# lazear/sage

Measured on NVIDIA H100. Metric: spectra/sec, higher is better.
Workload: dtype f32

## Files before the change

### sage_b200/csrc/device_common.cuh

```cuda
#pragma once
#include <cuda_runtime.h>
#include <stdint.h>

namespace sb {

constexpr int K_MAX = 128;
constexpr uint32_t NARROW_CAP = 8192;
constexpr int PRELIM_THREADS = 256;
constexpr int SCORE_THREADS = 128;
#ifndef SAGE_B200_SCORE_MIN_CTAS
#define SAGE_B200_SCORE_MIN_CTAS 10
#endif
constexpr int SCORE_MIN_CTAS = SAGE_B200_SCORE_MIN_CTAS;
#ifndef SAGE_B200_SCORE_TILE
#define SAGE_B200_SCORE_TILE 1024
#endif
#ifndef SAGE_B200_SCORE_UNROLL
#define SAGE_B200_SCORE_UNROLL 1
#endif
#ifndef SAGE_B200_SCORE_MIN_CTAS_SPLIT
#define SAGE_B200_SCORE_MIN_CTAS_SPLIT 11
#endif
constexpr int SCORE_MIN_CTAS_SPLIT = SAGE_B200_SCORE_MIN_CTAS_SPLIT;
constexpr uint32_t SCORE_UNROLL = SAGE_B200_SCORE_UNROLL;
constexpr uint32_t SCORE_TILE = SAGE_B200_SCORE_TILE;
constexpr int MAX_KINDS = 6;
constexpr uint32_t WARPQ_CAP = 1024;
constexpr int WARPQ_WARPS = 2;
constexpr int WARPQ_MIN_CTAS = 24;
constexpr uint32_t PEP_LUT_CELLS = 65536;
constexpr uint32_t BUCKET_LUT_CELLS = 32768;

constexpr float PROTON = 1.0072764f;
constexpr float NEUTRON = 1.00335f;

struct Tol { int kind; float lo, hi; };

__device__ __forceinline__ int f32_key(float x) {
// ... 209 lines not shown
```

### sage_b200/csrc/kernels.cuh

```cuda
#pragma once
#include <type_traits>

#include "device_common.cuh"
#include "glibc_log.cuh"

#ifndef SAGE_B200_RARE_NOINLINE
#define SAGE_B200_RARE_NOINLINE 0
#endif
#if SAGE_B200_RARE_NOINLINE
#define SB_RARE __noinline__
#else
#define SB_RARE __forceinline__
#endif

namespace sb {

__device__ __forceinline__ uint32_t pep_partition(const DbView& db, float x, bool le) {
    uint32_t lo = 0, hi = db.n_pep;
    if (db.pep_lut != nullptr) {
        const float t = (x - db.plut_base) * db.plut_inv_w;
        if (t == t) {
            const int c = (int)fminf(fmaxf(floorf(t), -2.0f), (float)PEP_LUT_CELLS + 2.0f);
            lo = __ldg(db.pep_lut + min(max(c - 1, 0), (int)PEP_LUT_CELLS));
            hi = __ldg(db.pep_lut + min(max(c + 2, 0), (int)PEP_LUT_CELLS));
// ... 1294 lines not shown
    const int klo = f32_key(lo), khi = f32_key(hi);
    uint32_t i, j;
    binary_search_slice(n, [&](uint32_t k) { return f32_key(masses[k]) < klo; }, [&](uint32_t k) { return f32_key(masses[k]) <= khi; }, i, j);
    int best = -1;
    float max_int = 0.0f;
    for (uint32_t idx = i; idx < j; idx++) {
        const float m = masses[idx];
        if (m >= lo && m <= hi) {
            const float it = intens[idx];
            if (it >= max_int) { max_int = it; best = (int)idx; }
        }
    }
    return best;
}
__device__ __forceinline__ int select_most_intense_peak_lut(const float* masses, const float* intens, uint32_t n, float center, const Tol& tol,
                                                            const LutParams& LP, const uint16_t* lut) {
    float lo, hi;
    tol_bounds(tol, center, lo, hi);
    lo = __fadd_rn(lo, 0.0f);
    hi = __fadd_rn(hi, 0.0f);
    uint32_t idx = lut_start(LP, lut, lo, SPEC_LUT_CELLS);
    while (idx < n && masses[idx] < lo) idx++;
    int best = -1;
    float max_int = 0.0f;
    while (idx < n) {
        const float m = masses[idx];
        if (!(m <= hi)) break;
        const float it = intens[idx];
        if (it >= max_int) { max_int = it; best = (int)idx; }
        idx++;
    }
    return best;
}

__device__ __forceinline__ double ref_ln(const ScorerView& sc, double x) { return glog::glibc_log_v(x, (int)sc.log_variant); }
__device__ __forceinline__ double lnfact(const ScorerView& sc, uint32_t n) {
// ... 150 lines not shown

__device__ __forceinline__ unsigned long long f64_sort_key(double d) {
    const unsigned long long u = (unsigned long long)__double_as_longlong(d + 0.0);
    return (u >> 63) ? ~u : (u | 0x8000000000000000ull);
}
__device__ __forceinline__ double f64_from_sort_key(unsigned long long k) {
    const unsigned long long u = (k >> 63) ? (k & 0x7FFFFFFFFFFFFFFFull) : ~k;
    return __longlong_as_double((long long)u);
}

#if SAGE_B200_PHASE_CLOCKS
__device__ unsigned long long g_phase[16];
__shared__ long long s_ph_prev;
#define PH_START() do { if (threadIdx.x == 0) s_ph_prev = clock64(); } while (0)
#define PH(i) do { if (threadIdx.x == 0) { const long long n_ = clock64(); atomicAdd(&g_phase[i], (unsigned long long)(n_ - s_ph_prev)); s_ph_prev = n_; } } while (0)
#else
#define PH_START() do {} while (0)
#define PH(i) do {} while (0)
#endif

struct ScoreTile {
    CandHdr hdr[K_MAX + 1];
    double hkey[K_MAX];
    float term[SCORE_TILE];
    float inten[SCORE_TILE];
    uint32_t mask[SCORE_TILE / 32];
    uint16_t hits[SCORE_TILE];
    uint16_t lut[SPEC_LUT_CELLS];
    uint32_t scan[SCORE_THREADS / 32];
    unsigned long long hit_base;
    uint32_t hit_room;
};

__device__ __forceinline__ uint32_t kind_index(uint32_t ki, uint32_t nions) {
    uint32_t kind = ki >= nions;
    uint32_t idx = ki - (kind ? nions : 0);
    while (idx >= nions) { idx -= nions; kind++; }
    return kind << 13 | idx;
}

__device__ __forceinline__ bool fast_task(float ion, uint32_t fc, float tlo, float thi, const SpecView& sp, const uint16_t* lut, const float* pm, float& mz,
                                          uint32_t& idx) {
    const float q3 = __fmul_rn(ion, 1.0f / 3.0f);
    const float third = __fmaf_rn(__fmaf_rn(-q3, 3.0f, ion), 1.0f / 3.0f, q3);
    mz = fc == 1 ? ion : (fc == 2 ? __fmul_rn(ion, 0.5f) : third);
    const float pl = __fmul_rn(mz, tlo), ph = __fmul_rn(mz, thi);
    const float ql = __fmul_rn(pl, 1.0f / 1000000.0f), qh = __fmul_rn(ph, 1.0f / 1000000.0f);
    const float lo = __fadd_rn(mz, __fmaf_rn(__fmaf_rn(-ql, 1000000.0f, pl), 1.0f / 1000000.0f, ql));
    const float hi = __fadd_rn(mz, __fmaf_rn(__fmaf_rn(-qh, 1000000.0f, ph), 1.0f / 1000000.0f, qh));
    const float tt = __fmul_rn(__fsub_rn(lo, sp.lp.base), sp.lp.inv_w);
    const int cc = tt > 1.0f ? (int)fminf(tt, (float)(SPEC_LUT_CELLS - 1)) - 1 : 0;
    idx = lut[cc];
    while (pm[idx] < lo) idx++;
    return pm[idx] <= hi;
}

template <bool FAST, bool SPLIT>
__device__ __forceinline__ void score_candidates_flat(const DbView& db, const ScorerView& sc, const uint64_t* cur, uint32_t ncand, const SpecView& sp,
                                                      ScoreTile& S, ScoreRec* recs, const SplitOut& so, uint32_t spec) {
    const uint32_t tid = threadIdx.x, lane = tid & 31, warp = tid >> 5, nwarps = SCORE_THREADS / 32;
    constexpr uint32_t tile = SCORE_TILE;
    uint64_t key = 0;
    uint32_t L = 0, nions = 0, nfc = 1, total = 0, ion_off = 0;
    if (tid < ncand) {
        key = cur[tid];
        const uint32_t pep = key_peptide(key);
        L = __ldg(db.pep_len + pep);
        nions = L - 1;
        nfc = max_fragment_charge(sc.max_fragment_charge_opt, key_charge(key)) - 1;
        total = nions * nfc * db.n_kinds;
        ion_off = __ldg(db.ion_off + pep);
    }
    uint32_t incl = total;
#pragma unroll
    for (int o = 1; o < 32; o <<= 1) {
        const uint32_t v = __shfl_up_sync(0xffffffffu, incl, o);
        if (lane >= (uint32_t)o) incl += v;
    }
    if (lane == 31) S.scan[warp] = incl;
    __syncthreads();
    uint32_t base = incl - total, T = 0;
#pragma unroll
    for (uint32_t w = 0; w < nwarps; w++) {
        const uint32_t x = S.scan[w];
        if (w < warp) base += x;
        T += x;
    }
    if (tid < ncand) { CandHdr h; h.ion_off = ion_off; h.base = base; h.next = base + total; h.nions = (uint16_t)nions; h.nfc = (uint8_t)nfc; h.pad = 0; S.hdr[tid] = h; }
    if (tid == 0) { CandHdr h; h.ion_off = 0; h.base = T; h.next = 0xFFFFFFFFu; h.nions = 0; h.nfc = 1; h.pad = 0; S.hdr[ncand] = h; }
    uint32_t hcnt = 0, hits_before = 0;
    if (SPLIT && tid == 0) {
        const unsigned long long hb = atomicAdd(so.counters + C_HITS, (unsigned long long)T);
        const bool room = hb + T <= so.hit_cap;
        S.hit_base = hb;
        S.hit_room = room ? 1u : 0u;
        so.meta[spec].hit_base = hb;
        if (!room) so.meta[spec].ncand = 0;
    }
    uint32_t mb = 0, my = 0;
    float sb = 0.f, sy = 0.f, ppm = 0.f;
    Run brun = {0, 0, 0, 0}, yrun = {0, 0, 0, 0};
    const float tlo = sc.fragment_tol.lo, thi = sc.fragment_tol.hi;
    const float* const pm = sp.masses;
    const float* const pi = sp.intens;
    auto generic_task = [&](const CandHdr& h, uint32_t f, uint32_t slot) -> bool {
        uint32_t ki, fc;
        switch (h.nfc) {
            case 1: ki = f; fc = 1; break;
            case 2: ki = f >> 1; fc = (f & 1) + 1; break;
            case 3: ki = f / 3; fc = f - ki * 3 + 1; break;
            default: ki = f / h.nfc; fc = f - ki * h.nfc + 1; break;
        }
        const float ion = __ldg(db.ions + h.ion_off + ki);
        const float mz = fc == 1 ? ion : (fc == 2 && fabsf(ion) >= 1e-30f) ? __fmul_rn(ion, 0.5f) : __fdiv_rn(ion, (float)fc);
        const int pk = sp.use_lut ? select_most_intense_peak_lut(pm, pi, sp.np, mz, sc.fragment_tol, sp.lp, S.lut)
                                  : select_most_intense_peak(pm, pi, sp.np, mz, sc.fragment_tol);
        if (pk < 0) return false;
        const float peak_mass = pm[pk], inten = pi[pk];
        S.term[slot] = __fdiv_rn(__fmul_rn(__fmul_rn(inten, fabsf(__fsub_rn(mz, peak_mass))), 2E6f), __fadd_rn(mz, peak_mass));
        S.inten[slot] = inten;
        return true;
    };
    for (uint32_t t0 = 0; t0 < T; t0 += tile) {
        const uint32_t tn = min(tile, T - t0);
        __syncthreads();
        PH(t0 == 0 ? 3 : 5);
        constexpr uint32_t STEP = 32 * SCORE_UNROLL;
        const uint32_t chunk = (((tn + nwarps - 1) / nwarps) + STEP - 1) & ~(STEP - 1);
        const uint32_t w_lo = min(tn, warp * chunk), w_hi = min(tn, w_lo + chunk);
        uint32_t c = 0, wcount = 0;
        CandHdr h = S.hdr[0];
        if (w_lo < w_hi) {
            const uint32_t t_first = t0 + min(w_lo + lane, w_hi - 1);
            uint32_t lo = 0, hi = ncand;
            while (hi - lo > 1) { const uint32_t mid = (lo + hi) >> 1; if (S.hdr[mid].base <= t_first) lo = mid; else hi = mid; }
            c = lo;
            h = S.hdr[c];
// ... 15 lines not shown
                hB = h; fB = t - h.base;
            }
            if (FAST) {
                const bool okA = inA && hA.nfc <= 3, okB = inB && hB.nfc <= 3;
                const uint32_t kiA = hA.nfc == 1 ? fA : (hA.nfc == 2 ? fA >> 1 : __umulhi(fA, 0xAAAAAAABu) >> 1);
                const uint32_t kiB = hB.nfc == 1 ? fB : (hB.nfc == 2 ? fB >> 1 : __umulhi(fB, 0xAAAAAAABu) >> 1);
                const float ionA = okA ? __ldg(db.ions + hA.ion_off + kiA) : 0.0f;
                const float ionB = okB ? __ldg(db.ions + hB.ion_off + kiB) : 0.0f;
                const bool fastA = okA && ionA >= 1.0f && ionA <= 1e20f, fastB = okB && ionB >= 1.0f && ionB <= 1e20f;
                float mzA = 0.f, mzB = 0.f;
                uint32_t idxA = 0, idxB = 0;
                if (fastA) hitA = fast_task(ionA, fA - kiA * hA.nfc + 1, tlo, thi, sp, S.lut, pm, mzA, idxA);
                if (fastB) hitB = fast_task(ionB, fB - kiB * hB.nfc + 1, tlo, thi, sp, S.lut, pm, mzB, idxB);
                if (hitA) { S.term[slotA] = mzA; S.inten[slotA] = __uint_as_float(idxA); }
                if (hitB) { S.term[slotB] = mzB; S.inten[slotB] = __uint_as_float(idxB); }
                if (inA && !fastA) hitA = finalA = generic_task(hA, fA, slotA);
                if (inB && !fastB) hitB = finalB = generic_task(hB, fB, slotB);
            } else {
                if (inA) hitA = generic_task(hA, fA, slotA);
                if (inB) hitB = generic_task(hB, fB, slotB);
            }
            const uint32_t ballA = __ballot_sync(0xffffffffu, hitA), ballB = __ballot_sync(0xffffffffu, hitB);
            if (lane == 0) { S.mask[s0 >> 5] = ballA; if (SCORE_UNROLL == 2) S.mask[(s0 >> 5) + 1] = ballB; }
            if (FAST) {
                const uint32_t lt = (1u << lane) - 1;
                if (hitA) S.hits[w_lo + wcount + __popc(ballA & lt)] = (uint16_t)(slotA | (finalA ? 0x8000u : 0u));
                wcount += __popc(ballA);
                if (SCORE_UNROLL == 2) {
                    if (hitB) S.hits[w_lo + wcount + __popc(ballB & lt)] = (uint16_t)(slotB | (finalB ? 0x8000u : 0u));
                    wcount += __popc(ballB);
                }
            }
        }
        if (FAST) {
            __syncwarp();
// ... 12 lines not shown
                    const float it = pi[idx];
                    if (it >= max_int) { max_int = it; best = (int)idx; }
                    m = pm[++idx];
                } while (m <= hi);
                if (best >= 0) {
                    const float peak_mass = pm[best];
                    S.term[slot] = __fdiv_rn(__fmul_rn(__fmul_rn(max_int, fabsf(__fsub_rn(mz, peak_mass))), 2E6f), __fadd_rn(mz, peak_mass));
                    S.inten[slot] = max_int;
                } else {
                    atomicAnd(&S.mask[slot >> 5], ~(1u << (slot & 31)));
                }
            }
        }
        __syncthreads();
        PH(4);
        if (SPLIT) {
            const uint32_t nwords = (tn + 31) >> 5;
            const uint32_t mw = lane < nwords ? S.mask[lane] : 0u;
            uint32_t incl = (uint32_t)__popc(mw);
#pragma unroll
            for (int o = 1; o < 32; o <<= 1) {
                const uint32_t v = __shfl_up_sync(0xffffffffu, incl, o);
                if (lane >= (uint32_t)o) incl += v;
            }
            const uint32_t pre = incl - (uint32_t)__popc(mw), tile_total = __shfl_sync(0xffffffffu, incl, 31);
            const uint32_t word = tid >> 2, q8 = (tid & 3) * 8;
            const uint32_t wm = word < nwords ? S.mask[word] : 0u;
            const uint32_t p = __shfl_sync(0xffffffffu, pre, word & 31);
            uint32_t m8 = (wm >> q8) & 0xFFu;
            const bool room = S.hit_room != 0;
            while (m8) {
                const uint32_t bit = q8 + (uint32_t)__ffs(m8) - 1;
                m8 &= m8 - 1;
                const uint32_t slot = (word << 5) + bit, t = t0 + slot;
                uint32_t lo = 0, hi = ncand;
                while (hi - lo > 1) { const uint32_t mid = (lo + hi) >> 1; if (S.hdr[mid].base <= t) lo = mid; else hi = mid; }
                while (t >= S.hdr[lo].next) lo++;
                const CandHdr hh = S.hdr[lo];
                const uint32_t f = t - hh.base;
                const uint32_t ki = hh.nfc == 1 ? f : (hh.nfc == 2 ? f >> 1 : f / hh.nfc);
                if (room) {
                    const unsigned long long g = S.hit_base + hits_before + p + (uint32_t)__popc(wm & ((1u << bit) - 1u));
                    so.hit_k[g] = (uint16_t)kind_index(ki, hh.nions);
                    so.hit_i[g] = S.inten[slot];
                    so.hit_t[g] = S.term[slot];
                }
            }
            if (tid < ncand && total) {
                const uint32_t a = max(base, t0), b = min(base + total, t0 + tn);
                if (a < b) {
                    const uint32_t sa = a - t0, se = b - t0 - 1;
                    for (uint32_t w = sa >> 5; w <= se >> 5; w++) {
                        uint32_t m = S.mask[w];
                        if (w == sa >> 5) m &= 0xffffffffu << (sa & 31);
                        if (w == se >> 5) m &= 0xffffffffu >> (31 - (se & 31));
                        hcnt += (uint32_t)__popc(m);
                    }
                }
            }
            hits_before += tile_total;
            continue;
        }
        if (tid < ncand && total) {
            const uint32_t a = max(base, t0), b = min(base + total, t0 + tn);
            if (a < b) {
                const uint32_t sa = a - t0, se = b - t0 - 1;
                for (uint32_t w = sa >> 5; w <= se >> 5; w++) {
                    uint32_t m = S.mask[w];
                    if (w == sa >> 5) m &= 0xffffffffu << (sa & 31);
                    if (w == se >> 5) m &= 0xffffffffu >> (31 - (se & 31));
                    while (m) {
                        const uint32_t slot = (w << 5) + (uint32_t)__ffs(m) - 1;
                        m &= m - 1;
                        const uint32_t f = t0 + slot - base;
                        uint32_t ki;
                        switch (nfc) {
                            case 1: ki = f; break;
// ... 1 lines not shown
                            case 3: ki = f / 3; break;
                            default: ki = f / nfc; break;
                        }
                        uint32_t kind_i = ki >= nions;
                        uint32_t idx = ki - (kind_i ? nions : 0);
                        while (idx >= nions) { idx -= nions; kind_i++; }
                        const float it = S.inten[slot];
                        ppm = __fadd_rn(ppm, S.term[slot]);
                        if ((db.nterm_mask >> kind_i) & 1) { mb++; sb = __fadd_rn(sb, it); brun.matched(idx); }
                        else { my++; sy = __fadd_rn(sy, it); yrun.matched(idx); }
                    }
                }
            }
        }
    }
    if (SPLIT) {
        uint32_t inc2 = hcnt;
#pragma unroll
        for (int o = 1; o < 32; o <<= 1) {
            const uint32_t v = __shfl_up_sync(0xffffffffu, inc2, o);
            if (lane >= (uint32_t)o) inc2 += v;
        }
        __syncthreads();
        if (lane == 31) S.scan[warp] = inc2;
        __syncthreads();
        uint32_t h0 = inc2 - hcnt;
#pragma unroll
        for (uint32_t w = 0; w < nwarps; w++) if (w < warp) h0 += S.scan[w];
        if (tid < ncand) {
            CandOut co;
            co.key = key; co.h0 = h0; co.hcnt = hcnt; co.nions = (uint16_t)nions; co.nfc = (uint8_t)nfc; co.plen = (uint8_t)L; co.pad = 0;
            so.cand[(size_t)spec * sc.kparam + tid] = co;
        }
        return;
    }
    if (tid < ncand) {
        ScoreRec r;
        r.peptide = key_peptide(key); r.charge = key_charge(key); r.iso = key_iso(key);
        r.matched_b = mb & 0xFFFF; r.matched_y = my & 0xFFFF; r.summed_b = sb; r.summed_y = sy;
        r.longest_b = brun.longest; r.longest_y = yrun.longest;
        r.hyperscore = hyperscore_of(sc, r.matched_b, r.matched_y, sb, sy);
        r.ppm_difference = __fdiv_rn(ppm, __fadd_rn(sb, sy));
        r.valid = ((r.matched_b + r.matched_y) & 0xFFFF) >= sc.min_matched_peaks;
        r.plen = L;
        recs[tid] = r;
        S.hkey[tid] = r.valid ? r.hyperscore : -INFINITY;
    }
}

__device__ SB_RARE void annotate_candidate_warp(const DbView& db, const ScorerView& sc, uint32_t pep, uint32_t charge, const SpecView& sp,
// ... 39 lines not shown
}

__device__ __forceinline__ bool spectrum_lut_setup(const float* masses , uint32_t np, uint16_t* lut, LutParams& lp) {
    bool bad = np == 0 || np >= 65536;
    for (uint32_t i = threadIdx.x; i < np; i += blockDim.x) {
        const float m = masses[i];
        bad |= !(m > 0.0f) || (i > 0 && !(m >= masses[i - 1]));
    }
    if (__syncthreads_or(bad)) return false;
    lp = lut_params(masses[0], masses[np - 1], SPEC_LUT_CELLS);
    lut_build_walk(masses, np, lp, lut, threadIdx.x, blockDim.x, SPEC_LUT_CELLS);
    __syncthreads();
    return true;
}

template <bool SPLIT>
__global__ void __launch_bounds__(SCORE_THREADS, SPLIT ? SCORE_MIN_CTAS_SPLIT : SCORE_MIN_CTAS) k_score(DbView db, ScorerView sc, BatchView b, FeatureOut* features, uint32_t* counts, uint32_t pmax,
                                                         uint64_t* dbg_keys , uint32_t* dbg_meta, FragmentOut* frag_out ,
                                                         unsigned long long frag_cap, uint32_t quick_mode ,
                                                         uint8_t* keep , SplitOut so) {
    extern __shared__ __align__(16) unsigned char smem_raw[];
    float* masses_raw = reinterpret_cast<float*>(smem_raw);
    float* intens_raw = masses_raw + pmax + 4;
    uint64_t* cur = reinterpret_cast<uint64_t*>(intens_raw + pmax + 4);
    uint64_t* tot = cur + sc.lcap;
    ScoreRec* recs = reinterpret_cast<ScoreRec*>(tot + sc.lcap);
    uint32_t* order = reinterpret_cast<uint32_t*>(recs + sc.kparam);
    uint8_t* mark = reinterpret_cast<uint8_t*>(order + sc.kparam);
    __shared__ __align__(16) ScoreTile S;
    uint16_t* const lut = S.lut;
    __shared__ uint32_t s_ntot, s_ncand, s_np, s_nvalid;
    __shared__ unsigned long long s_matched_peaks, s_scored;
    __shared__ float s_tic;

    const uint32_t s = b.order ? b.order[blockIdx.x] : blockIdx.x, tid = threadIdx.x, lane = tid & 31, warp = tid >> 5, nwarps = SCORE_THREADS / 32;
// ... 70 lines not shown
            if (key_peptide(tot[i]) != 0xFFFFFFFFu) cur[nc++] = tot[i];
        s_ncand = nc;
        s_np = np;
        s_tic = b.tic[s];
    }
    __syncthreads();
    PH(0);
    if (dbg_keys != nullptr) {
        for (uint32_t i = tid; i < s_ntot; i += SCORE_THREADS) dbg_keys[(size_t)s * sc.kparam + i] = tot[i];
        if (tid == 0) { dbg_meta[s * 4 + 0] = s_ntot; dbg_meta[s * 4 + 1] = (uint32_t)s_matched_peaks; dbg_meta[s * 4 + 2] = (uint32_t)s_scored; }
    }
    if (np) mbar_wait(&s_bar, 0);
    PH(1);
    if (tid == 0) masses[np] = INFINITY;
    const uint32_t ncand = s_ncand;
    if (SPLIT && tid == 0) {
        SpecMeta m;
        m.hit_base = 0; m.matched_peaks = s_matched_peaks; m.scored = s_scored; m.ncand = ncand; m.pad = 0;
        so.meta[s] = m;
    }
    const bool lists_fit = b.counters[C_NLIST_NEED] <= b.nlist_cap && b.counters[C_WIDE] <= (unsigned long long)b.wide_cap;
    if (quick_mode != 0 && !lists_fit) return;
    if (quick_mode == 1) {
        for (uint32_t i = tid; i < ncand; i += SCORE_THREADS) keep[key_peptide(cur[i])] = 1;
        return;
    }
    const float mzp = __fsub_rn(b.prec_mz[s], PROTON);
    const double lambda = (double)s_matched_peaks / (double)s_scored;
    const uint32_t rounds = sc.chimera ? sc.report_psms : 1;
    const uint32_t per_round = sc.chimera ? 1 : sc.report_psms;
    uint32_t nout = 0;
    SpecView sv;
    sv.masses = masses; sv.intens = intens; sv.lut = lut;
    for (uint32_t round = 0; round < rounds && ncand; round++) {
        np = s_np;
        sv.np = np;
        sv.use_lut = spectrum_lut_setup(masses, np, lut, sv.lp);
        PH(2);
        if (tid == 0) s_nvalid = 0;
        if (sv.use_lut && sc.score_fast && sc.fragment_tol.kind == 0 && fast_tol_ok(sc.fragment_tol.lo) && fast_tol_ok(sc.fragment_tol.hi))
            score_candidates_flat<true, SPLIT>(db, sc, cur, ncand, sv, S, recs, so, s);
        else
            score_candidates_flat<false, SPLIT>(db, sc, cur, ncand, sv, S, recs, so, s);
        if (SPLIT) return;
        __syncthreads();
        PH(5);
        if (quick_mode == 2) {
            if (tid < ncand && recs[tid].valid) {
                const uint32_t pme = recs[tid].peptide;
                uint32_t pos = 0;
                for (uint32_t j = 0; j < ncand; j++) {
                    if (!recs[j].valid) continue;
                    const uint32_t pj = recs[j].peptide;
                    pos += (pj > pme) || (pj == pme && j < tid);
                }
                if (pos < sc.report_psms) keep[pme] = 1;
            }
            return;
        }
// ... 104 lines not shown
            if (lane == 0) {
                float t = 0.0f;
                for (uint32_t i = 0; i < w; i++) t = __fadd_rn(t, intens[i]);
                s_tic = t;
                s_np = w;
                masses[w] = INFINITY;
            }
        }
        __syncthreads();
    }
    PH(6);
    if (tid == 0) {
        counts[s] = nout;
        if (nout) atomicAdd(b.counters + C_PSMS, (unsigned long long)nout);
    }
}

__global__ void __launch_bounds__(128) k_fold(DbView db, ScorerView sc, SplitOut so, uint32_t n) {
    __shared__ unsigned long long s_floats[4];
    const uint64_t i = (uint64_t)blockIdx.x * blockDim.x + threadIdx.x;
    const uint32_t s = (uint32_t)(i / sc.kparam), c = (uint32_t)(i - (uint64_t)s * sc.kparam);
    const bool me = s < n && c < so.meta[s].ncand;
    unsigned long long a_floats = me ? 2ull * so.cand[(size_t)s * sc.kparam + c].plen + 2ull : 0ull;
    for (int o = 16; o > 0; o >>= 1) a_floats += __shfl_down_sync(0xffffffffu, a_floats, o);
    if ((threadIdx.x & 31) == 0) s_floats[threadIdx.x >> 5] = a_floats;
    __syncthreads();
    if (threadIdx.x == 0) {
        const unsigned long long t = s_floats[0] + s_floats[1] + s_floats[2] + s_floats[3];
        if (t) atomicAdd(so.counters + C_PEPFLOATS, t);
    }
// ... 486 lines not shown
```

### sage_b200/csrc/sage_b200.cu

```cuda
#include <cub/device/device_radix_sort.cuh>
#include <cub/device/device_scan.cuh>
#include <cuda_runtime.h>

#include <pthread.h>
#include <sched.h>

#include <algorithm>
#include <atomic>
#include <cctype>
#include <cmath>
#include <cstdarg>
#include <cstdio>
#include <cstdlib>
#include <cstring>
#include <chrono>
#include <condition_variable>
#include <memory>
#include <mutex>
#include <thread>
#include <string>
#include <vector>

#include "../../include/sage_b200.h"
#include "kernels.cuh"
// ... 618 lines not shown
    static bool done[64] = {};
    std::lock_guard<std::mutex> lock(mu);
    if (device >= 0 && device < 64 && done[device]) return 0;
    int optin = 0;
    CUDA_TRY(cudaDeviceGetAttribute(&optin, cudaDevAttrMaxSharedMemoryPerBlockOptin, device));
    auto raise = [&](const void* fn) -> cudaError_t {
        cudaFuncAttributes fa;
        cudaError_t e = cudaFuncGetAttributes(&fa, fn);
        if (e != cudaSuccess) return e;
        return cudaFuncSetAttribute(fn, cudaFuncAttributeMaxDynamicSharedMemorySize, optin - (int)fa.sharedSizeBytes);
    };
    CUDA_TRY(raise((const void*)k_prelim_narrow));
    CUDA_TRY(raise((const void*)k_replay<true>));
    CUDA_TRY(raise((const void*)k_replay<false>));
    CUDA_TRY(raise((const void*)k_prelim_wide));
    CUDA_TRY(raise((const void*)k_score<false>));
    CUDA_TRY(raise((const void*)k_score<true>));
    CUDA_TRY(raise((const void*)k_process_ms2));
    if (device >= 0 && device < 64) done[device] = true;
    return 0;
}

extern "C" int sage_b200_host_log_variant(void) {
    static int cached = -2;
    if (cached != -2) return cached;
    uint64_t st = 0x9E3779B97F4A7C15ull;
    auto next = [&]() { st ^= st << 13; st ^= st >> 7; st ^= st << 17; return st; };
    bool ok[2] = {true, true};
    for (int i = 0; i < 6000; i++) {
        const uint64_t u = next();
        double x;
        switch (i % 3) {
// ... 540 lines not shown
    CUDA_TRY(cudaStreamWaitEvent(st, L.ev_intens, 0));
    const bool split = S->score_split && !sv.chimera && !annotate && !dbg && S->quick_mode == 0;
    if (split) {
        C.hits_cap = std::max<uint64_t>(C.force_hits, (uint64_t)std::ceil((S->hits_per_spectrum > 0.0 ? S->hits_per_spectrum : 4096.0) * (double)n) + 65536);
        if ((rc = L.d_cand.reserve((size_t)n * sv.kparam * sizeof(CandOut)))) return rc;
        if ((rc = L.d_meta.reserve((size_t)n * sizeof(SpecMeta)))) return rc;
        if ((rc = L.d_recs.reserve((size_t)n * sv.kparam * sizeof(ScoreRec)))) return rc;
        if ((rc = L.d_hkey.reserve((size_t)n * sv.kparam * 8))) return rc;
        if ((rc = L.d_emit.reserve((size_t)n * sv.report_psms * 4 + 16))) return rc;
        if ((rc = L.d_hitk.reserve(2 * C.hits_cap + 16))) return rc;
        if ((rc = L.d_hiti.reserve(4 * C.hits_cap + 16))) return rc;
        if ((rc = L.d_hitt.reserve(4 * C.hits_cap + 16))) return rc;
        SplitOut so{};
        so.cand = L.d_cand.as<CandOut>(); so.meta = L.d_meta.as<SpecMeta>(); so.hit_k = L.d_hitk.as<uint16_t>(); so.hit_i = L.d_hiti.as<float>();
        so.hit_t = L.d_hitt.as<float>(); so.hit_cap = C.hits_cap; so.recs = L.d_recs.as<ScoreRec>(); so.hkey = L.d_hkey.as<unsigned long long>(); so.counters = bv.counters;
        const size_t smem_split = (size_t)(C.pmax + 4) * 8 + (size_t)sv.lcap * 16 + 32;
        k_score<true><<<n, SCORE_THREADS, smem_split, st>>>(db->v, sv, bv, L.d_features.as<FeatureOut>(), L.d_counts.as<uint32_t>(), C.pmax, nullptr, nullptr, nullptr, 0ull, 0u,
                                                            nullptr, so);
        CUDA_TRY(cudaGetLastError());
        const uint64_t nthr = (uint64_t)n * sv.kparam, nrow = (uint64_t)n * sv.report_psms;
        CUDA_TRY(cudaMemsetAsync(L.d_emit.p, 0xFF, 4 * nrow, st));
        k_fold<<<(unsigned)((nthr + 127) / 128), 128, 0, st>>>(db->v, sv, so, n);
        CUDA_TRY(cudaGetLastError());
        k_features<<<(unsigned)((nthr + 127) / 128), 128, 0, st>>>(sv, n, so, L.d_emit.as<uint32_t>());
        CUDA_TRY(cudaGetLastError());
        k_rows<<<(unsigned)((nrow + 127) / 128), 128, 0, st>>>(db->v, sv, bv, so, L.d_emit.as<uint32_t>(), L.d_counts.as<uint32_t>(), L.d_features.as<FeatureOut>());
        CUDA_TRY(cudaGetLastError());
        launches += 4;
    } else {
        C.hits_cap = 0;
        k_score<false><<<n, SCORE_THREADS, C.smem, st>>>(db->v, sv, bv, L.d_features.as<FeatureOut>(), L.d_counts.as<uint32_t>(), C.pmax,
                                                        dbg ? L.d_dbgk.as<uint64_t>() : nullptr, dbg ? L.d_dbgm.as<uint32_t>() : nullptr,
                                                        annotate ? L.d_frags.as<FragmentOut>() : nullptr, (unsigned long long)S->frag_cap, S->quick_mode,
                                                        S->d_keep.as<uint8_t>(), SplitOut{});
        CUDA_TRY(cudaGetLastError());
        launches++;
    }
    CUDA_TRY(cudaEventRecord(L.ev[4], st));
    CUDA_TRY(cudaMemcpyAsync(L.h_counters.p, L.d_counters.p, 8 * C_COUNT, cudaMemcpyDeviceToHost, st));
    L.launches = launches;
    L.dbg = dbg;
    L.ran = true;
    return 0;
}

static int chunk_download(sage_b200_scorer* S, Lane& L, sage_b200_feature* fdst, uint32_t* cdst) {
    const ScorerView& sv = S->sv;
    cudaStream_t st = L.stream;
    ChunkState& C = L.chunk;
// ... 627 lines not shown
```

Baseline: 23.11 million.

## Replace split-mode k_score with warp-per-spectrum k_match kernel

Removes the SPLIT path from k_score and adds a dedicated k_match kernel in which each warp handles one spectrum, packing several warps per CTA within a 64KB shared-memory budget. Each warp builds a smaller peak LUT (512 cells) and runs per-warp queues to resolve fragment matches. Hits are streamed straight to the global hit arrays. The aim is to avoid CTA-wide __syncthreads and idle threads when spectra have few candidates, in exchange for less parallelism per spectrum and a coarser LUT.

```diff
diff --git a/sage_b200/csrc/device_common.cuh b/sage_b200/csrc/device_common.cuh
--- a/sage_b200/csrc/device_common.cuh
+++ b/sage_b200/csrc/device_common.cuh
@@ -18,10 +18,20 @@
 #ifndef SAGE_B200_SCORE_UNROLL
 #define SAGE_B200_SCORE_UNROLL 1
 #endif
-#ifndef SAGE_B200_SCORE_MIN_CTAS_SPLIT
-#define SAGE_B200_SCORE_MIN_CTAS_SPLIT 11
-#endif
-constexpr int SCORE_MIN_CTAS_SPLIT = SAGE_B200_SCORE_MIN_CTAS_SPLIT;
+#ifndef SAGE_B200_MATCH_LUT_CELLS
+#define SAGE_B200_MATCH_LUT_CELLS 512
+#endif
+#ifndef SAGE_B200_MATCH_MIN_CTAS
+#define SAGE_B200_MATCH_MIN_CTAS 10
+#endif
+#ifndef SAGE_B200_MATCH_UNROLL
+#define SAGE_B200_MATCH_UNROLL 2
+#endif
+constexpr uint32_t MATCH_UNROLL = SAGE_B200_MATCH_UNROLL;
+constexpr int MATCH_MIN_CTAS = SAGE_B200_MATCH_MIN_CTAS;
+constexpr uint32_t MATCH_WARPS = 4;
+constexpr size_t MATCH_CTA_SMEM = 64 * 1024;
+constexpr uint32_t MATCH_LUT_CELLS = SAGE_B200_MATCH_LUT_CELLS;
 constexpr uint32_t SCORE_UNROLL = SAGE_B200_SCORE_UNROLL;
 constexpr uint32_t SCORE_TILE = SAGE_B200_SCORE_TILE;
 constexpr int MAX_KINDS = 6;
diff --git a/sage_b200/csrc/kernels.cuh b/sage_b200/csrc/kernels.cuh
--- a/sage_b200/csrc/kernels.cuh
+++ b/sage_b200/csrc/kernels.cuh
@@ -1332,12 +1332,12 @@
     return best;
 }
 __device__ __forceinline__ int select_most_intense_peak_lut(const float* masses, const float* intens, uint32_t n, float center, const Tol& tol,
-                                                            const LutParams& LP, const uint16_t* lut) {
+                                                            const LutParams& LP, const uint16_t* lut, uint32_t cells = SPEC_LUT_CELLS) {
     float lo, hi;
     tol_bounds(tol, center, lo, hi);
     lo = __fadd_rn(lo, 0.0f);
     hi = __fadd_rn(hi, 0.0f);
-    uint32_t idx = lut_start(LP, lut, lo, SPEC_LUT_CELLS);
+    uint32_t idx = lut_start(LP, lut, lo, cells);
     while (idx < n && masses[idx] < lo) idx++;
     int best = -1;
     float max_int = 0.0f;
@@ -1518,9 +1518,15 @@
 __shared__ long long s_ph_prev;
 #define PH_START() do { if (threadIdx.x == 0) s_ph_prev = clock64(); } while (0)
 #define PH(i) do { if (threadIdx.x == 0) { const long long n_ = clock64(); atomicAdd(&g_phase[i], (unsigned long long)(n_ - s_ph_prev)); s_ph_prev = n_; } } while (0)
+__shared__ long long s_ph_warp[32];
+#define PH_WARP_START() do { if ((threadIdx.x & 31) == 0) s_ph_warp[threadIdx.x >> 5] = clock64(); } while (0)
+#define PH_WARP(i) do { if ((threadIdx.x & 31) == 0) { const long long n_ = clock64(); atomicAdd(&g_phase[i], (unsigned long long)(n_ - s_ph_warp[threadIdx.x >> 5])); \
+                                                       s_ph_warp[threadIdx.x >> 5] = n_; } } while (0)
 #else
 #define PH_START() do {} while (0)
 #define PH(i) do {} while (0)
+#define PH_WARP_START() do {} while (0)
+#define PH_WARP(i) do {} while (0)
 #endif
 
 struct ScoreTile {
@@ -1532,8 +1538,6 @@
     uint16_t hits[SCORE_TILE];
     uint16_t lut[SPEC_LUT_CELLS];
     uint32_t scan[SCORE_THREADS / 32];
-    unsigned long long hit_base;
-    uint32_t hit_room;
 };
 
 __device__ __forceinline__ uint32_t kind_index(uint32_t ki, uint32_t nions) {
@@ -1543,6 +1547,7 @@
     return kind << 13 | idx;
 }
 
+template <uint32_t CELLS = SPEC_LUT_CELLS>
 __device__ __forceinline__ bool fast_task(float ion, uint32_t fc, float tlo, float thi, const SpecView& sp, const uint16_t* lut, const float* pm, float& mz,
                                           uint32_t& idx) {
     const float q3 = __fmul_rn(ion, 1.0f / 3.0f);
@@ -1553,15 +1558,35 @@
     const float lo = __fadd_rn(mz, __fmaf_rn(__fmaf_rn(-ql, 1000000.0f, pl), 1.0f / 1000000.0f, ql));
     const float hi = __fadd_rn(mz, __fmaf_rn(__fmaf_rn(-qh, 1000000.0f, ph), 1.0f / 1000000.0f, qh));
     const float tt = __fmul_rn(__fsub_rn(lo, sp.lp.base), sp.lp.inv_w);
-    const int cc = tt > 1.0f ? (int)fminf(tt, (float)(SPEC_LUT_CELLS - 1)) - 1 : 0;
+    const int cc = tt > 1.0f ? (int)fminf(tt, (float)(CELLS - 1)) - 1 : 0;
     idx = lut[cc];
     while (pm[idx] < lo) idx++;
     return pm[idx] <= hi;
 }
 
-template <bool FAST, bool SPLIT>
+template <uint32_t CELLS = SPEC_LUT_CELLS>
+__device__ __forceinline__ bool generic_task(const DbView& db, const ScorerView& sc, const SpecView& sp, const CandHdr& h, uint32_t f, float& term, float& inten) {
+    uint32_t ki, fc;
+    switch (h.nfc) {
+        case 1: ki = f; fc = 1; break;
+        case 2: ki = f >> 1; fc = (f & 1) + 1; break;
+        case 3: ki = f / 3; fc = f - ki * 3 + 1; break;
+        default: ki = f / h.nfc; fc = f - ki * h.nfc + 1; break;
+    }
+    const float ion = __ldg(db.ions + h.ion_off + ki);
+    const float mz = fc == 1 ? ion : (fc == 2 && fabsf(ion) >= 1e-30f) ? __fmul_rn(ion, 0.5f) : __fdiv_rn(ion, (float)fc);
+    const int pk = sp.use_lut ? select_most_intense_peak_lut(sp.masses, sp.intens, sp.np, mz, sc.fragment_tol, sp.lp, sp.lut, CELLS)
+                              : select_most_intense_peak(sp.masses, sp.intens, sp.np, mz, sc.fragment_tol);
+    if (pk < 0) return false;
+    const float peak_mass = sp.masses[pk];
+    inten = sp.intens[pk];
+    term = __fdiv_rn(__fmul_rn(__fmul_rn(inten, fabsf(__fsub_rn(mz, peak_mass))), 2E6f), __fadd_rn(mz, peak_mass));
+    return true;
+}
+
+template <bool FAST>
 __device__ __forceinline__ void score_candidates_flat(const DbView& db, const ScorerView& sc, const uint64_t* cur, uint32_t ncand, const SpecView& sp,
-                                                      ScoreTile& S, ScoreRec* recs, const SplitOut& so, uint32_t spec) {
+                                                      ScoreTile& S, ScoreRec* recs) {
     const uint32_t tid = threadIdx.x, lane = tid & 31, warp = tid >> 5, nwarps = SCORE_THREADS / 32;
     constexpr uint32_t tile = SCORE_TILE;
     uint64_t key = 0;
@@ -1592,39 +1617,13 @@
     }
     if (tid < ncand) { CandHdr h; h.ion_off = ion_off; h.base = base; h.next = base + total; h.nions = (uint16_t)nions; h.nfc = (uint8_t)nfc; h.pad = 0; S.hdr[tid] = h; }
     if (tid == 0) { CandHdr h; h.ion_off = 0; h.base = T; h.next = 0xFFFFFFFFu; h.nions = 0; h.nfc = 1; h.pad = 0; S.hdr[ncand] = h; }
-    uint32_t hcnt = 0, hits_before = 0;
-    if (SPLIT && tid == 0) {
-        const unsigned long long hb = atomicAdd(so.counters + C_HITS, (unsigned long long)T);
-        const bool room = hb + T <= so.hit_cap;
-        S.hit_base = hb;
-        S.hit_room = room ? 1u : 0u;
-        so.meta[spec].hit_base = hb;
-        if (!room) so.meta[spec].ncand = 0;
-    }
     uint32_t mb = 0, my = 0;
     float sb = 0.f, sy = 0.f, ppm = 0.f;
     Run brun = {0, 0, 0, 0}, yrun = {0, 0, 0, 0};
     const float tlo = sc.fragment_tol.lo, thi = sc.fragment_tol.hi;
     const float* const pm = sp.masses;
     const float* const pi = sp.intens;
-    auto generic_task = [&](const CandHdr& h, uint32_t f, uint32_t slot) -> bool {
-        uint32_t ki, fc;
-        switch (h.nfc) {
-            case 1: ki = f; fc = 1; break;
-            case 2: ki = f >> 1; fc = (f & 1) + 1; break;
-            case 3: ki = f / 3; fc = f - ki * 3 + 1; break;
-            default: ki = f / h.nfc; fc = f - ki * h.nfc + 1; break;
-        }
-        const float ion = __ldg(db.ions + h.ion_off + ki);
-        const float mz = fc == 1 ? ion : (fc == 2 && fabsf(ion) >= 1e-30f) ? __fmul_rn(ion, 0.5f) : __fdiv_rn(ion, (float)fc);
-        const int pk = sp.use_lut ? select_most_intense_peak_lut(pm, pi, sp.np, mz, sc.fragment_tol, sp.lp, S.lut)
-                                  : select_most_intense_peak(pm, pi, sp.np, mz, sc.fragment_tol);
-        if (pk < 0) return false;
-        const float peak_mass = pm[pk], inten = pi[pk];
-        S.term[slot] = __fdiv_rn(__fmul_rn(__fmul_rn(inten, fabsf(__fsub_rn(mz, peak_mass))), 2E6f), __fadd_rn(mz, peak_mass));
-        S.inten[slot] = inten;
-        return true;
-    };
+    auto generic_slot = [&](const CandHdr& h, uint32_t f, uint32_t slot) -> bool { return generic_task(db, sc, sp, h, f, S.term[slot], S.inten[slot]); };
     for (uint32_t t0 = 0; t0 < T; t0 += tile) {
         const uint32_t tn = min(tile, T - t0);
         __syncthreads();
@@ -1670,11 +1669,11 @@
                 if (fastB) hitB = fast_task(ionB, fB - kiB * hB.nfc + 1, tlo, thi, sp, S.lut, pm, mzB, idxB);
                 if (hitA) { S.term[slotA] = mzA; S.inten[slotA] = __uint_as_float(idxA); }
                 if (hitB) { S.term[slotB] = mzB; S.inten[slotB] = __uint_as_float(idxB); }
-                if (inA && !fastA) hitA = finalA = generic_task(hA, fA, slotA);
-                if (inB && !fastB) hitB = finalB = generic_task(hB, fB, slotB);
+                if (inA && !fastA) hitA = finalA = generic_slot(hA, fA, slotA);
+                if (inB && !fastB) hitB = finalB = generic_slot(hB, fB, slotB);
             } else {
-                if (inA) hitA = generic_task(hA, fA, slotA);
-                if (inB) hitB = generic_task(hB, fB, slotB);
+                if (inA) hitA = generic_slot(hA, fA, slotA);
+                if (inB) hitB = generic_slot(hB, fB, slotB);
             }
             const uint32_t ballA = __ballot_sync(0xffffffffu, hitA), ballB = __ballot_sync(0xffffffffu, hitB);
             if (lane == 0) { S.mask[s0 >> 5] = ballA; if (SCORE_UNROLL == 2) S.mask[(s0 >> 5) + 1] = ballB; }
@@ -1717,53 +1716,6 @@
         }
         __syncthreads();
         PH(4);
-        if (SPLIT) {
-            const uint32_t nwords = (tn + 31) >> 5;
-            const uint32_t mw = lane < nwords ? S.mask[lane] : 0u;
-            uint32_t incl = (uint32_t)__popc(mw);
-#pragma unroll
-            for (int o = 1; o < 32; o <<= 1) {
-                const uint32_t v = __shfl_up_sync(0xffffffffu, incl, o);
-                if (lane >= (uint32_t)o) incl += v;
-            }
-            const uint32_t pre = incl - (uint32_t)__popc(mw), tile_total = __shfl_sync(0xffffffffu, incl, 31);
-            const uint32_t word = tid >> 2, q8 = (tid & 3) * 8;
-            const uint32_t wm = word < nwords ? S.mask[word] : 0u;
-            const uint32_t p = __shfl_sync(0xffffffffu, pre, word & 31);
-            uint32_t m8 = (wm >> q8) & 0xFFu;
-            const bool room = S.hit_room != 0;
-            while (m8) {
-                const uint32_t bit = q8 + (uint32_t)__ffs(m8) - 1;
-                m8 &= m8 - 1;
-                const uint32_t slot = (word << 5) + bit, t = t0 + slot;
-                uint32_t lo = 0, hi = ncand;
-                while (hi - lo > 1) { const uint32_t mid = (lo + hi) >> 1; if (S.hdr[mid].base <= t) lo = mid; else hi = mid; }
-                while (t >= S.hdr[lo].next) lo++;
-                const CandHdr hh = S.hdr[lo];
-                const uint32_t f = t - hh.base;
-                const uint32_t ki = hh.nfc == 1 ? f : (hh.nfc == 2 ? f >> 1 : f / hh.nfc);
-                if (room) {
-                    const unsigned long long g = S.hit_base + hits_before + p + (uint32_t)__popc(wm & ((1u << bit) - 1u));
-                    so.hit_k[g] = (uint16_t)kind_index(ki, hh.nions);
-                    so.hit_i[g] = S.inten[slot];
-                    so.hit_t[g] = S.term[slot];
-                }
-            }
-            if (tid < ncand && total) {
-                const uint32_t a = max(base, t0), b = min(base + total, t0 + tn);
-                if (a < b) {
-                    const uint32_t sa = a - t0, se = b - t0 - 1;
-                    for (uint32_t w = sa >> 5; w <= se >> 5; w++) {
-                        uint32_t m = S.mask[w];
-                        if (w == sa >> 5) m &= 0xffffffffu << (sa & 31);
-                        if (w == se >> 5) m &= 0xffffffffu >> (31 - (se & 31));
-                        hcnt += (uint32_t)__popc(m);
-                    }
-                }
-            }
-            hits_before += tile_total;
-            continue;
-        }
         if (tid < ncand && total) {
             const uint32_t a = max(base, t0), b = min(base + total, t0 + tn);
             if (a < b) {
@@ -1795,26 +1747,6 @@
             }
         }
     }
-    if (SPLIT) {
-        uint32_t inc2 = hcnt;
-#pragma unroll
-        for (int o = 1; o < 32; o <<= 1) {
-            const uint32_t v = __shfl_up_sync(0xffffffffu, inc2, o);
-            if (lane >= (uint32_t)o) inc2 += v;
-        }
-        __syncthreads();
-        if (lane == 31) S.scan[warp] = inc2;
-        __syncthreads();
-        uint32_t h0 = inc2 - hcnt;
-#pragma unroll
-        for (uint32_t w = 0; w < nwarps; w++) if (w < warp) h0 += S.scan[w];
-        if (tid < ncand) {
-            CandOut co;
-            co.key = key; co.h0 = h0; co.hcnt = hcnt; co.nions = (uint16_t)nions; co.nfc = (uint8_t)nfc; co.plen = (uint8_t)L; co.pad = 0;
-            so.cand[(size_t)spec * sc.kparam + tid] = co;
-        }
-        return;
-    }
     if (tid < ncand) {
         ScoreRec r;
         r.peptide = key_peptide(key); r.charge = key_charge(key); r.iso = key_iso(key);
@@ -1884,11 +1816,10 @@
     return true;
 }
 
-template <bool SPLIT>
-__global__ void __launch_bounds__(SCORE_THREADS, SPLIT ? SCORE_MIN_CTAS_SPLIT : SCORE_MIN_CTAS) k_score(DbView db, ScorerView sc, BatchView b, FeatureOut* features, uint32_t* counts, uint32_t pmax,
+__global__ void __launch_bounds__(SCORE_THREADS, SCORE_MIN_CTAS) k_score(DbView db, ScorerView sc, BatchView b, FeatureOut* features, uint32_t* counts, uint32_t pmax,
                                                          uint64_t* dbg_keys , uint32_t* dbg_meta, FragmentOut* frag_out ,
                                                          unsigned long long frag_cap, uint32_t quick_mode ,
-                                                         uint8_t* keep , SplitOut so) {
+                                                         uint8_t* keep ) {
     extern __shared__ __align__(16) unsigned char smem_raw[];
     float* masses_raw = reinterpret_cast<float*>(smem_raw);
     float* intens_raw = masses_raw + pmax + 4;
@@ -1989,11 +1920,6 @@
     PH(1);
     if (tid == 0) masses[np] = INFINITY;
     const uint32_t ncand = s_ncand;
-    if (SPLIT && tid == 0) {
-        SpecMeta m;
-        m.hit_base = 0; m.matched_peaks = s_matched_peaks; m.scored = s_scored; m.ncand = ncand; m.pad = 0;
-        so.meta[s] = m;
-    }
     const bool lists_fit = b.counters[C_NLIST_NEED] <= b.nlist_cap && b.counters[C_WIDE] <= (unsigned long long)b.wide_cap;
     if (quick_mode != 0 && !lists_fit) return;
     if (quick_mode == 1) {
@@ -2014,10 +1940,9 @@
         PH(2);
         if (tid == 0) s_nvalid = 0;
         if (sv.use_lut && sc.score_fast && sc.fragment_tol.kind == 0 && fast_tol_ok(sc.fragment_tol.lo) && fast_tol_ok(sc.fragment_tol.hi))
-            score_candidates_flat<true, SPLIT>(db, sc, cur, ncand, sv, S, recs, so, s);
+            score_candidates_flat<true>(db, sc, cur, ncand, sv, S, recs);
         else
-            score_candidates_flat<false, SPLIT>(db, sc, cur, ncand, sv, S, recs, so, s);
-        if (SPLIT) return;
+            score_candidates_flat<false>(db, sc, cur, ncand, sv, S, recs);
         __syncthreads();
         PH(5);
         if (quick_mode == 2) {
@@ -2152,6 +2077,315 @@
         counts[s] = nout;
         if (nout) atomicAdd(b.counters + C_PSMS, (unsigned long long)nout);
     }
+}
+
+constexpr uint32_t MATCH_QUEUE = 64;
+struct MatchLayout { uint32_t off_i, off_cur, off_bar, off_scr, off_lut, off_qa, off_qb, off_qm, off_hc, bytes; };
+__host__ __device__ inline MatchLayout match_layout(uint32_t pmax, uint32_t lcap, uint32_t kparam) {
+    MatchLayout m;
+    m.off_i = (pmax + 4) * 4;
+    m.off_cur = 2 * m.off_i;
+    m.off_bar = m.off_cur + ((lcap * 8 + 15) & ~15u);
+    m.off_scr = m.off_bar + 16;
+    m.off_lut = m.off_scr + (kparam + 1) * (uint32_t)sizeof(CandHdr);
+    m.off_qa = m.off_lut + MATCH_LUT_CELLS * 2;
+    m.off_qb = m.off_qa + MATCH_QUEUE * 4;
+    m.off_qm = m.off_qb + MATCH_QUEUE * 4;
+    m.off_hc = m.off_qm + MATCH_QUEUE * 4;
+    const uint32_t scr = m.off_hc + kparam * 4 - m.off_scr;
+    m.bytes = (m.off_scr + (scr > lcap * 8 ? scr : lcap * 8) + 15) & ~15u;
+    return m;
+}
+static_assert(MATCH_LUT_CELLS % 8 == 0 && MATCH_LUT_CELLS >= 64, "k_match LUT size");
+
+template <bool FAST>
+__device__ __forceinline__ void match_tasks(const DbView& db, const ScorerView& sc, const SpecView& sp, const CandHdr* hdr, uint32_t T, float* qa,
+                                            uint32_t* qb, uint32_t* qm, uint32_t* hc, const SplitOut& so, unsigned long long g0) {
+    const uint32_t lane = threadIdx.x & 31, lt = (1u << lane) - 1;
+    const float tlo = sc.fragment_tol.lo, thi = sc.fragment_tol.hi;
+    const float* const pm = sp.masses;
+    const float* const pi = sp.intens;
+    uint32_t qhead = 0, qtail = 0, written = 0;
+    auto resolve = [&](uint32_t cnt) {
+        __syncwarp();
+        bool valid = false;
+        float term = 0.f, inten = 0.f;
+        uint32_t m = 0;
+        if (lane < cnt) {
+            const uint32_t e = (qhead + lane) & (MATCH_QUEUE - 1);
+            m = qm[e];
+            const float a = qa[e];
+            const uint32_t bb = qb[e];
+            if (!FAST || (m >> 31)) {
+                valid = true; term = a; inten = __uint_as_float(bb);
+            } else {
+                const float mz = a;
+                uint32_t idx = bb;
+                const float ph = __fmul_rn(mz, thi), qh = __fmul_rn(ph, 1.0f / 1000000.0f);
+                const float hi = __fadd_rn(mz, __fmaf_rn(__fmaf_rn(-qh, 1000000.0f, ph), 1.0f / 1000000.0f, qh));
+                int best = -1;
+                float max_int = 0.0f;
+                float pmv;
+                do {
+                    const float it = pi[idx];
+                    if (it >= max_int) { max_int = it; best = (int)idx; }
+                    pmv = pm[++idx];
+                } while (pmv <= hi);
+                if (best >= 0) {
+                    const float peak_mass = pm[best];
+                    term = __fdiv_rn(__fmul_rn(__fmul_rn(max_int, fabsf(__fsub_rn(mz, peak_mass))), 2E6f), __fadd_rn(mz, peak_mass));
+                    inten = max_int;
+                    valid = true;
+                }
+            }
+        }
+        const uint32_t vb = __ballot_sync(0xffffffffu, valid);
+        if (valid) {
+            const unsigned long long g = g0 + written + (uint32_t)__popc(vb & lt);
+            so.hit_k[g] = (uint16_t)m;
+            so.hit_i[g] = inten;
+            so.hit_t[g] = term;
+            atomicAdd(hc + ((m >> 16) & 0xFFu), 1u);
+        }
+        written += (uint32_t)__popc(vb);
+        qhead += cnt;
+        __syncwarp();
+    };
+    uint32_t c = 0;
+    CandHdr h = hdr[0];
+    constexpr uint32_t U = MATCH_UNROLL;
+    for (uint32_t t0 = 0; t0 < T; t0 += 32 * U) {
+        CandHdr hh[U];
+        uint32_t f[U], cc[U], ki3[U];
+        bool in[U];
+        float ion[U];
+#pragma unroll
+        for (uint32_t u = 0; u < U; u++) {
+            const uint32_t t = t0 + 32 * u + lane;
+            in[u] = t < T;
+            f[u] = 0;
+            if (in[u]) {
+                while (t >= h.next) { c++; h = hdr[c]; }
+                f[u] = t - h.base;
+            }
+            hh[u] = h;
+            cc[u] = c;
+            ki3[u] = h.nfc == 1 ? f[u] : (h.nfc == 2 ? f[u] >> 1 : __umulhi(f[u], 0xAAAAAAABu) >> 1);
+            ion[u] = FAST && in[u] && h.nfc <= 3 ? __ldg(db.ions + h.ion_off + ki3[u]) : 0.0f;
+        }
+#pragma unroll
+        for (uint32_t u = 0; u < U; u++) {
+            bool hit = false, fin = false;
+            float a = 0.f, it = 0.f;
+            uint32_t bb = 0;
+            if (FAST) {
+                const bool fst = in[u] && hh[u].nfc <= 3 && ion[u] >= 1.0f && ion[u] <= 1e20f;
+                if (fst) hit = fast_task<MATCH_LUT_CELLS>(ion[u], f[u] - ki3[u] * hh[u].nfc + 1, tlo, thi, sp, sp.lut, pm, a, bb);
+                else if (in[u]) { hit = fin = generic_task<MATCH_LUT_CELLS>(db, sc, sp, hh[u], f[u], a, it); bb = __float_as_uint(it); }
+            } else if (in[u]) {
+                hit = fin = generic_task<MATCH_LUT_CELLS>(db, sc, sp, hh[u], f[u], a, it);
+                bb = __float_as_uint(it);
+            }
+            const uint32_t ball = __ballot_sync(0xffffffffu, hit);
+            if (hit) {
+                const uint32_t ki = hh[u].nfc <= 3 ? ki3[u] : f[u] / hh[u].nfc;
+                const uint32_t e = (qtail + (uint32_t)__popc(ball & lt)) & (MATCH_QUEUE - 1);
+                qa[e] = a;
+                qb[e] = bb;
+                qm[e] = (fin ? 0x80000000u : 0u) | cc[u] << 16 | kind_index(ki, hh[u].nions);
+            }
+            qtail += (uint32_t)__popc(ball);
+            if (qtail - qhead >= 32) {
+                PH_WARP(4);
+                resolve(32);
+                PH_WARP(5);
+            }
+        }
+    }
+    PH_WARP(4);
+    if (qtail != qhead) resolve(qtail - qhead);
+    PH_WARP(5);
+}
+
+__global__ void __launch_bounds__(MATCH_WARPS * 32, MATCH_MIN_CTAS) k_match(DbView db, ScorerView sc, BatchView b, uint32_t pmax, SplitOut so) {
+    extern __shared__ __align__(16) unsigned char smem_raw[];
+    const uint32_t lane = threadIdx.x & 31, warp = threadIdx.x >> 5, lt = (1u << lane) - 1;
+    const uint32_t i = blockIdx.x * (blockDim.x >> 5) + warp;
+    if (i >= b.n) return;
+    const uint32_t s = b.order ? b.order[i] : i;
+    PH_WARP_START();
+    const MatchLayout ml = match_layout(pmax, sc.lcap, sc.kparam);
+    unsigned char* const base = smem_raw + (size_t)warp * ml.bytes;
+    float* const masses_raw = reinterpret_cast<float*>(base);
+    float* const intens_raw = reinterpret_cast<float*>(base + ml.off_i);
+    uint64_t* const cur = reinterpret_cast<uint64_t*>(base + ml.off_cur);
+    uint64_t* const bar = reinterpret_cast<uint64_t*>(base + ml.off_bar);
+    uint64_t* const tot = reinterpret_cast<uint64_t*>(base + ml.off_scr);
+    CandHdr* const hdr = reinterpret_cast<CandHdr*>(base + ml.off_scr);
+    uint16_t* const lut = reinterpret_cast<uint16_t*>(base + ml.off_lut);
+    uint32_t* const hc = reinterpret_cast<uint32_t*>(base + ml.off_hc);
+
+    const uint32_t p0 = b.peak_off[s];
+    const uint32_t np = b.peak_off[s + 1] - p0;
+    const uint32_t a0 = p0 & ~3u, head = p0 - a0;
+    const uint32_t bytes = ((head + np) * 4 + 15) & ~15u;
+    float* const masses = masses_raw + head;
+    float* const intens = intens_raw + head;
+    if (lane == 0) {
+        mbar_init(bar, 1);
+        if (np) {
+            mbar_arrive_expect_tx(bar, 2 * bytes);
+            bulk_copy_g2s(masses_raw, b.masses + a0, bytes, bar);
+            bulk_copy_g2s(intens_raw, b.intens + a0, bytes, bar);
+        }
+    }
+
+    const QueryDesc* qd = b.queries + (size_t)s * sc.qmax;
+    const QueryHits* qh = b.hits + (size_t)s * sc.qmax;
+    const uint64_t* qk = b.hit_keys + (size_t)s * sc.qmax * sc.kparam;
+    const bool iso_fold = sc.min_iso != sc.max_iso;
+    const bool single = !iso_fold && (sc.qmax == 1 || qd[1].mode == 0) && qd[0].mode != 0;
+    uint32_t ncand = 0;
+    unsigned long long mp = 0, scd = 0;
+    if (single) {
+        const QueryHits h = qh[0];
+        const uint32_t n = h.n ? h.n : min(h.default_run, sc.kparam);
+        for (uint32_t j0 = 0; j0 < n; j0 += 32) {
+            const uint32_t j = j0 + lane;
+            const uint64_t k = (j < n && h.n) ? qk[j] : PRESCORE_DEFAULT;
+            const bool keep = j < n && key_peptide(k) != 0xFFFFFFFFu;
+            const uint32_t ball = __ballot_sync(0xffffffffu, keep);
+            if (keep) cur[ncand + (uint32_t)__popc(ball & lt)] = k;
+            ncand += (uint32_t)__popc(ball);
+        }
+        mp = h.matched_peaks;
+        scd = h.scored_candidates;
+    } else {
+        if (lane == 0) {
+            uint32_t ntot = 0, nq = 0;
+            while (nq < sc.qmax && qd[nq].mode != 0) nq++;
+            const uint32_t nch = sc.n_iso ? nq / sc.n_iso : 0;
+            for (uint32_t ci = 0; ci < nch; ci++) {
+                uint32_t ncur = 0;
+                for (uint32_t ii = 0; ii < sc.n_iso; ii++) {
+                    const uint32_t qi = ci * sc.n_iso + ii;
+                    mp += qh[qi].matched_peaks;
+                    scd += qh[qi].scored_candidates;
+                    ncur = append_hits(cur, ncur, sc.lcap, qh[qi], qk + (size_t)qi * sc.kparam, sc.kparam);
+                }
+                if (iso_fold) {
+                    const uint32_t k = min(ncur, sc.kparam);
+                    bounded_min_heapify_seq(cur, ncur, k);
+                    ncur = k;
+                }
+                for (uint32_t j = 0; j < ncur && ntot < sc.lcap; j++) tot[ntot++] = cur[j];
+            }
+            {
+                const uint32_t k = min(ntot, sc.kparam);
+                bounded_min_heapify_seq(tot, ntot, k);
+                ntot = k;
+            }
+            for (uint32_t j = 0; j < ntot; j++)
+                if (key_peptide(tot[j]) != 0xFFFFFFFFu) cur[ncand++] = tot[j];
+        }
+        ncand = __shfl_sync(0xffffffffu, ncand, 0);
+        mp = __shfl_sync(0xffffffffu, mp, 0);
+        scd = __shfl_sync(0xffffffffu, scd, 0);
+    }
+    __syncwarp();
+    PH_WARP(0);
+    if (np) mbar_wait(bar, 0);
+    PH_WARP(1);
+    if (lane == 0) masses[np] = INFINITY;
+    __syncwarp();
+    if (ncand == 0) {
+        if (lane == 0) { SpecMeta m; m.hit_base = 0; m.matched_peaks = mp; m.scored = scd; m.ncand = 0; m.pad = 0; so.meta[s] = m; }
+        return;
+    }
+
+    SpecView sv;
+    sv.masses = masses; sv.intens = intens; sv.np = np; sv.lut = lut;
+    bool bad = np == 0 || np >= 65536;
+    for (uint32_t j = lane; j < np; j += 32) {
+        const float m = masses[j];
+        bad |= !(m > 0.0f) || (j > 0 && !(m >= masses[j - 1]));
+    }
+    sv.use_lut = !__any_sync(0xffffffffu, bad);
+    if (sv.use_lut) {
+        sv.lp = lut_params(masses[0], masses[np - 1], MATCH_LUT_CELLS);
+        lut_build_walk(masses, np, sv.lp, lut, lane, 32, MATCH_LUT_CELLS);
+    }
+    PH_WARP(2);
+
+    const uint32_t per = (ncand + 31) >> 5;
+    uint32_t sum = 0;
+    for (uint32_t q = 0; q < per; q++) {
+        const uint32_t j = lane * per + q;
+        if (j < ncand) {
+            const uint64_t key = cur[j];
+            const uint32_t pep = key_peptide(key);
+            const uint32_t L = __ldg(db.pep_len + pep);
+            const uint32_t nions = L - 1;
+            const uint32_t nfc = max_fragment_charge(sc.max_fragment_charge_opt, key_charge(key)) - 1;
+            const uint32_t total = nions * nfc * db.n_kinds;
+            CandHdr hh; hh.ion_off = __ldg(db.ion_off + pep); hh.base = 0; hh.next = total; hh.nions = (uint16_t)nions; hh.nfc = (uint8_t)nfc; hh.pad = (uint8_t)L;
+            hdr[j] = hh;
+            hc[j] = 0;
+            sum += total;
+        }
+    }
+    uint32_t incl = sum;
+#pragma unroll
+    for (int o = 1; o < 32; o <<= 1) {
+        const uint32_t v = __shfl_up_sync(0xffffffffu, incl, o);
+        if (lane >= (uint32_t)o) incl += v;
+    }
+    const uint32_t T = __shfl_sync(0xffffffffu, incl, 31);
+    uint32_t run = incl - sum;
+    for (uint32_t q = 0; q < per; q++) {
+        const uint32_t j = lane * per + q;
+        if (j < ncand) { const uint32_t tot_j = hdr[j].next; hdr[j].base = run; hdr[j].next = run + tot_j; run += tot_j; }
+    }
+    if (lane == 0) { CandHdr hh; hh.ion_off = 0; hh.base = T; hh.next = 0xFFFFFFFFu; hh.nions = 0; hh.nfc = 1; hh.pad = 0; hdr[ncand] = hh; }
+    unsigned long long hb = 0;
+    if (lane == 0) {
+        hb = atomicAdd(so.counters + C_HITS, (unsigned long long)T);
+        SpecMeta m; m.hit_base = hb; m.matched_peaks = mp; m.scored = scd; m.ncand = hb + T <= so.hit_cap ? ncand : 0; m.pad = 0;
+        so.meta[s] = m;
+    }
+    hb = __shfl_sync(0xffffffffu, hb, 0);
+    if (hb + T > so.hit_cap) return;
+    __syncwarp();
+    PH_WARP(3);
+
+    if (sv.use_lut && sc.score_fast && sc.fragment_tol.kind == 0 && fast_tol_ok(sc.fragment_tol.lo) && fast_tol_ok(sc.fragment_tol.hi))
+        match_tasks<true>(db, sc, sv, hdr, T, reinterpret_cast<float*>(base + ml.off_qa), reinterpret_cast<uint32_t*>(base + ml.off_qb),
+                          reinterpret_cast<uint32_t*>(base + ml.off_qm), hc, so, hb);
+    else
+        match_tasks<false>(db, sc, sv, hdr, T, reinterpret_cast<float*>(base + ml.off_qa), reinterpret_cast<uint32_t*>(base + ml.off_qb),
+                           reinterpret_cast<uint32_t*>(base + ml.off_qm), hc, so, hb);
+    __syncwarp();
+
+    sum = 0;
+    for (uint32_t q = 0; q < per; q++) { const uint32_t j = lane * per + q; if (j < ncand) sum += hc[j]; }
+    incl = sum;
+#pragma unroll
+    for (int o = 1; o < 32; o <<= 1) {
+        const uint32_t v = __shfl_up_sync(0xffffffffu, incl, o);
+        if (lane >= (uint32_t)o) incl += v;
+    }
+    run = incl - sum;
+    for (uint32_t q = 0; q < per; q++) {
+        const uint32_t j = lane * per + q;
+        if (j < ncand) {
+            const CandHdr hh = hdr[j];
+            CandOut co;
+            co.key = cur[j]; co.h0 = run; co.hcnt = hc[j]; co.nions = hh.nions; co.nfc = hh.nfc; co.plen = hh.pad; co.pad = 0;
+            so.cand[(size_t)s * sc.kparam + j] = co;
+            run += co.hcnt;
+        }
+    }
+    PH_WARP(6);
 }
 
 __global__ void __launch_bounds__(128) k_fold(DbView db, ScorerView sc, SplitOut so, uint32_t n) {
diff --git a/sage_b200/csrc/sage_b200.cu b/sage_b200/csrc/sage_b200.cu
--- a/sage_b200/csrc/sage_b200.cu
+++ b/sage_b200/csrc/sage_b200.cu
@@ -656,8 +656,8 @@
     CUDA_TRY(raise((const void*)k_replay<true>));
     CUDA_TRY(raise((const void*)k_replay<false>));
     CUDA_TRY(raise((const void*)k_prelim_wide));
-    CUDA_TRY(raise((const void*)k_score<false>));
-    CUDA_TRY(raise((const void*)k_score<true>));
+    CUDA_TRY(raise((const void*)k_score));
+    CUDA_TRY(raise((const void*)k_match));
     CUDA_TRY(raise((const void*)k_process_ms2));
     if (device >= 0 && device < 64) done[device] = true;
     return 0;
@@ -1228,9 +1228,10 @@
         SplitOut so{};
         so.cand = L.d_cand.as<CandOut>(); so.meta = L.d_meta.as<SpecMeta>(); so.hit_k = L.d_hitk.as<uint16_t>(); so.hit_i = L.d_hiti.as<float>();
         so.hit_t = L.d_hitt.as<float>(); so.hit_cap = C.hits_cap; so.recs = L.d_recs.as<ScoreRec>(); so.hkey = L.d_hkey.as<unsigned long long>(); so.counters = bv.counters;
-        const size_t smem_split = (size_t)(C.pmax + 4) * 8 + (size_t)sv.lcap * 16 + 32;
-        k_score<true><<<n, SCORE_THREADS, smem_split, st>>>(db->v, sv, bv, L.d_features.as<FeatureOut>(), L.d_counts.as<uint32_t>(), C.pmax, nullptr, nullptr, nullptr, 0ull, 0u,
-                                                            nullptr, so);
+        const uint32_t slice = match_layout(C.pmax, sv.lcap, sv.kparam).bytes;
+        uint32_t W = MATCH_WARPS;
+        while (W > 1 && (size_t)W * slice > MATCH_CTA_SMEM) W >>= 1;
+        k_match<<<(n + W - 1) / W, 32 * W, (size_t)W * slice, st>>>(db->v, sv, bv, C.pmax, so);
         CUDA_TRY(cudaGetLastError());
         const uint64_t nthr = (uint64_t)n * sv.kparam, nrow = (uint64_t)n * sv.report_psms;
         CUDA_TRY(cudaMemsetAsync(L.d_emit.p, 0xFF, 4 * nrow, st));
@@ -1243,10 +1244,10 @@
         launches += 4;
     } else {
         C.hits_cap = 0;
-        k_score<false><<<n, SCORE_THREADS, C.smem, st>>>(db->v, sv, bv, L.d_features.as<FeatureOut>(), L.d_counts.as<uint32_t>(), C.pmax,
+        k_score<<<n, SCORE_THREADS, C.smem, st>>>(db->v, sv, bv, L.d_features.as<FeatureOut>(), L.d_counts.as<uint32_t>(), C.pmax,
                                                         dbg ? L.d_dbgk.as<uint64_t>() : nullptr, dbg ? L.d_dbgm.as<uint32_t>() : nullptr,
                                                         annotate ? L.d_frags.as<FragmentOut>() : nullptr, (unsigned long long)S->frag_cap, S->quick_mode,
-                                                        S->d_keep.as<uint8_t>(), SplitOut{});
+                                                        S->d_keep.as<uint8_t>());
         CUDA_TRY(cudaGetLastError());
         launches++;
     }
```

Result: faster. 24.84 million, median of 6 (+7.5%).
